# leospeidel/Colate

Measured on AMD Instinct MI355X. Metric: bootstrap replicates/sec to EM convergence, whole-genome SGDP mut, 20 epochs, higher is better.
Workload: dtype f64

## Files before the change

### colate_amd/csrc/em_kernel_impl.hpp

```cpp
#pragma once
#include <hip/hip_runtime.h>

#include <cstdlib>
#include <cstring>
#include <type_traits>

#include "em_kernels.h"
#include "em_math.hpp"

namespace {

constexpr int kWave = 64;
enum { O_W = 0, O_N, O_D, kNumBinArrays };
enum { G_LAM = 0, G_INV, G_XA, G_P, G_BETA, G_CS, G_S, G_PW, kNumGather };
constexpr int G_Q = kNumGather;
constexpr int num_gather_rows(int nch, bool tput) { return (nch >= 2 || !tput) ? kNumGather + 1 : kNumGather; }
constexpr int tail_scratch_arrays(int nch, bool tput) { return nch >= 2 ? (tput ? 3 : 6) : 0; }

__device__ __forceinline__ double readlane_d(double v, int lane) {
  int lo = __builtin_amdgcn_readlane(__double2loint(v), lane);
  int hi = __builtin_amdgcn_readlane(__double2hiint(v), lane);
  return __hiloint2double(hi, lo);
}

template <int CTRL, int ROW_MASK = 0xf, bool BOUND = false>
__device__ __forceinline__ double dpp_d(double old, double v) {
  int lo = __builtin_amdgcn_update_dpp(__double2loint(old), __double2loint(v), CTRL, ROW_MASK, 0xf, BOUND);
  int hi = __builtin_amdgcn_update_dpp(__double2hiint(old), __double2hiint(v), CTRL, ROW_MASK, 0xf, BOUND);
  return __hiloint2double(hi, lo);
}
constexpr int ROW_SHR1 = 0x111, ROW_SHR2 = 0x112, ROW_SHR4 = 0x114, ROW_SHR8 = 0x118;
constexpr int ROW_SHL1 = 0x101, ROW_SHL2 = 0x102, ROW_SHL4 = 0x104, ROW_SHL8 = 0x108;
constexpr int ROW_BCAST15 = 0x142, ROW_BCAST31 = 0x143, WAVE_SHR1 = 0x138, WAVE_SHL1 = 0x130;


__device__ __forceinline__ double wave_prefix_sum(double v, int rows = 4) {
  v += dpp_d<ROW_SHR1, 0xf, true>(0.0, v);
  v += dpp_d<ROW_SHR2, 0xf, true>(0.0, v);
  v += dpp_d<ROW_SHR4, 0xf, true>(0.0, v);
  v += dpp_d<ROW_SHR8, 0xf, true>(0.0, v);
  if (rows > 1) v += dpp_d<ROW_BCAST15, 0xa>(0.0, v);
  if (rows > 2) v += dpp_d<ROW_BCAST31, 0xc>(0.0, v);
  return v;
}
__device__ __forceinline__ double wave_suffix_sum(double v, int lane, int rows = 4) {
  v += dpp_d<ROW_SHL1, 0xf, true>(0.0, v);
  v += dpp_d<ROW_SHL2, 0xf, true>(0.0, v);
  v += dpp_d<ROW_SHL4, 0xf, true>(0.0, v);
  v += dpp_d<ROW_SHL8, 0xf, true>(0.0, v);
  if (rows > 1) {
    const double r1 = readlane_d(v, 16);
    double add = 0.0;
    if (rows > 2) {
      const double r2 = readlane_d(v, 32), r3 = readlane_d(v, 48);
      const double s23 = r2 + r3, s123 = r1 + s23;
      const int row = lane >> 4;
      add = row == 0 ? s123 : (row == 1 ? s23 : (row == 2 ? r3 : 0.0));
    } else {
      add = (lane >> 4) == 0 ? r1 : 0.0;
    }
    v = v + add;
  }
  return v;
}
__device__ __forceinline__ void wave_affine_scan(double& a, double& b, int rows = 4, const double* nosrc = nullptr) {
#define COLATE_AFF_STEP(CTRL, RM, BND, K)                                                                   \
  {                                                                                                         \
    const double as = nosrc ? dpp_d<CTRL, RM, true>(0.0, a) + nosrc[K] : dpp_d<CTRL, RM>(1.0, a);           \
    const double bs = dpp_d<CTRL, RM, BND>(0.0, b);                                                         \
    b = em::fma_(a, bs, b);                                                                                 \
    a = a * as;                                                                                             \
  }
  COLATE_AFF_STEP(ROW_SHR1, 0xf, true, 0)
  COLATE_AFF_STEP(ROW_SHR2, 0xf, true, 1)
  COLATE_AFF_STEP(ROW_SHR4, 0xf, true, 2)
  COLATE_AFF_STEP(ROW_SHR8, 0xf, true, 3)
#undef COLATE_AFF_STEP
  if (rows == 2) {
    const double bs = dpp_d<ROW_BCAST15, 0xa>(0.0, b);
    b = em::fma_(a, bs, b);
  }
#define COLATE_AFF_STEP2(CTRL, RM)                 \
  {                                                \
    const double as = dpp_d<CTRL, RM>(1.0, a);     \
    const double bs = dpp_d<CTRL, RM>(0.0, b);     \
    b = em::fma_(a, bs, b);                        \
    a = a * as;                                    \
  }
  if (rows > 2) COLATE_AFF_STEP2(ROW_BCAST15, 0xa)
  if (rows > 2) COLATE_AFF_STEP2(ROW_BCAST31, 0xc)
#undef COLATE_AFF_STEP2
}
constexpr int kAffSteps = 6;
__device__ __forceinline__ void wave_affine_scan_rates(double a, double (&am)[kAffSteps], int rows, const double* nosrc) {
  am[0] = a;
#define COLATE_AFF_STEP(CTRL, RM, K)                                                                        \
  {                                                                                                         \
    const double as = nosrc ? dpp_d<CTRL, RM, true>(0.0, a) + nosrc[K] : dpp_d<CTRL, RM>(1.0, a);           \
    a = a * as;                                                                                             \
    am[K + 1] = a;                                                                                          \
  }
  COLATE_AFF_STEP(ROW_SHR1, 0xf, 0)
  COLATE_AFF_STEP(ROW_SHR2, 0xf, 1)
  COLATE_AFF_STEP(ROW_SHR4, 0xf, 2)
// ... 16 lines not shown
  v = __builtin_fmax(v, dpp_d<ROW_SHL4, 0xf, true>(0.0, v));
  v = __builtin_fmax(v, dpp_d<ROW_SHL8, 0xf, true>(0.0, v));
  const double r1 = readlane_d(v, 16), r2 = readlane_d(v, 32), r3 = readlane_d(v, 48);
  const double m23 = __builtin_fmax(r2, r3), m123 = __builtin_fmax(r1, m23);
  const int row = lane >> 4;
  return __builtin_fmax(v, row == 0 ? m123 : (row == 1 ? m23 : (row == 2 ? r3 : 0.0)));
}
__device__ __forceinline__ double half_ulp_pos(double z) {
  const int ex = (__double2hiint(z) >> 20) & 0x7ff;
  return ex > 53 ? __hiloint2double((ex - 53) << 20, 0) : 0.0;
}

__device__ __forceinline__ double tail_hneg(double z, double& q) {
  const float a = __builtin_fminf(__builtin_fabsf((float)z), 30.0f);
  const float t = __builtin_amdgcn_rcpf(__builtin_fmaf(0.2316419f, a, 1.0f));
  float poly = __builtin_fmaf(t, 1.330274429f, -1.821255978f);
  poly = __builtin_fmaf(t, poly, 1.781477937f);
  poly = __builtin_fmaf(t, poly, -0.356563782f);
  poly = __builtin_fmaf(t, poly, 0.319381530f);
  poly = poly * t;
  const float phi = 0.3989422804f * __builtin_amdgcn_exp2f(-0.72134752f * (a * a));
  const float qa = phi * poly;
  const float base = __builtin_fmaxf(__builtin_fmaf(-a, qa, phi), 0.0f);
  q = z < 0.0 ? (double)(1.0f - qa) : (double)qa;
  return (z < 0.0 ? -z : 0.0) + (double)base;
}

#ifdef COLATE_EM_STAMPS
__device__ __forceinline__ unsigned long long stamp() {
  unsigned long long t;
  __builtin_amdgcn_sched_barrier(0);
  asm volatile("s_memtime %0\n\ts_waitcnt lgkmcnt(0)" : "=s"(t)::"memory");
  __builtin_amdgcn_sched_barrier(0);
  return t;
}
#define COLATE_STAMP(i)                     \
  {                                         \
    const unsigned long long now_ = stamp(); \
    st_acc[i] += now_ - st_prev;            \
    st_prev = now_;                         \
  }
#define COLATE_PSTAMP(i) pro_t[i] = stamp();
#else
#define COLATE_STAMP(i)
#define COLATE_PSTAMP(i)
#endif

#ifdef COLATE_ABL
#define COLATE_ABL_HAS(b) (((COLATE_ABL) >> (b)) & 1)
#else
#define COLATE_ABL_HAS(b) 0
#endif

#define COLATE_COLD() asm volatile("; cold path")
#define COLATE_STR2(x) #x
#define COLATE_STR(x) COLATE_STR2(x)

__device__ __forceinline__ bool finite_pos(double x) { return x > 0.0 && x < __builtin_inf(); }

__device__ __forceinline__ unsigned long long ballot64(bool p) { return __builtin_amdgcn_ballot_w64(p); }

__device__ __forceinline__ void wave_lds_fence() {
  __builtin_amdgcn_fence(__ATOMIC_RELEASE, "wavefront");
  __builtin_amdgcn_wave_barrier();
  __builtin_amdgcn_fence(__ATOMIC_ACQUIRE, "wavefront");
}

struct BinStat {
  double a_b, cnt, tk, tkn, dtk, da, db;
  double f1, f2, f4, f8;
  int kb, pos;
  bool live, last_bin, is_tail;
};
enum { BF_F1 = 1, BF_F2 = 2, BF_F4 = 4, BF_F8 = 8, BF_TAIL = 16, BF_INRANGE = 32, BF_KB_SHIFT = 8 };

constexpr int em_loop_pad(int mode, int nch, int erows, bool tput, int wpe) {
#ifdef COLATE_LOOP_PAD
  return (COLATE_LOOP_PAD) & 7;
#else
  (void)erows, (void)wpe;
  if (mode != 0) return 0;
#ifdef COLATE_EM_ILP_BUILD
  (void)tput;
  return nch == 1 ? (wpe == 2 ? 2 : 6) : 2;
#else
  (void)nch;
  if (!tput) return 6;
  return 4;
#endif
#endif
}

constexpr int em_loop_pad2(int mode, int nch, bool tput) {
#if defined(COLATE_EM_ILP_BUILD) && !defined(COLATE_LOOP_PAD)
  (void)mode, (void)nch, (void)tput;
  return -1;
#else
  (void)mode, (void)nch, (void)tput;
  return -1;
#endif
}

constexpr bool em_affine_split(int nch, bool tput, int wpe) {
#ifdef COLATE_AFFINE_SPLIT
  (void)nch, (void)tput, (void)wpe;
  return (COLATE_AFFINE_SPLIT) != 0;
#else
  return !tput && nch == 1 && wpe == 2;
#endif
}

template <int MODE, int NCH, int EROWS, bool TPUT, int WPE = 0>
__global__ __launch_bounds__(TPUT ? 2 * kWave : 2 * COLATE_EM_MAX_A, WPE ? WPE : ((NCH == 1) ? 3 : (NCH == 2 ? 2 : 1))) void em_kernel(ColateEmArgs p) {
  extern __shared__ double lds[];
  const int E = p.E, A = p.A;
  constexpr int EPAD = NCH * kWave;
  const int NBMAX = (A + kWave - 1) / kWave;
  const int AP = NBMAX * kWave;
  const int APZ = AP + 2;
  const int tid = threadIdx.x, lane = tid & 63;
  constexpr int kSlotShift = (NCH == 1) ? 0 : (NCH == 2 ? 1 : (NCH == 4 ? 2 : (NCH == 8 ? 3 : 4)));
  static_assert(NCH == 1 || NCH == 2 || NCH == 4 || NCH == 8 || NCH == 16, "NCH");
  auto ep_of = [&](int c) { return lane * NCH + c; };
  const int wave = __builtin_amdgcn_readfirstlane(tid >> 6);
  const int role = wave & 1;
  const int grp = wave >> 1;
  const int rep = blockIdx.x;

  double* s_t = lds;
  double* s_ep = s_t + EPAD + 1;
  constexpr int kRows = num_gather_rows(NCH, TPUT);
  double* s_out = s_ep + kRows * EPAD;
  double* s_nd = s_out + 2 * kNumBinArrays * APZ;
  double* s_cfail = s_nd + 4 * EPAD;
  double* s_cnt = s_cfail + 2 * APZ;
  double* s_ll = s_cnt + 2 * APZ;
  double* s_exptab = s_ll + 12;
  double* s_age = s_exptab + em::kExpTableDoubles;
  double* s_tscr = s_age + AP;
  int* s_kb = reinterpret_cast<int*>(s_tscr + tail_scratch_arrays(NCH, TPUT) * APZ);
  int* s_fail = s_kb + AP + 1;
  int* s_misc = s_fail + 8;
  int* s_bflags = s_misc + 4;

#ifdef COLATE_EM_TRACE
  unsigned long long trace_t0;
  asm volatile("s_memtime %0\n\ts_waitcnt lgkmcnt(0)" : "=s"(trace_t0)::"memory");
#endif
#ifdef COLATE_EM_STAMPS
  unsigned long long pro_t[10] = {0, 0, 0, 0, 0, 0, 0, 0, 0, 0};
#endif
  COLATE_PSTAMP(0)
  const double* epochs = p.epochs + (size_t)rep * p.epochs_stride;
  for (int i = tid; i < EPAD + 1; i += blockDim.x) s_t[i] = (i < E) ? epochs[i] : 0.0;
  for (int i = tid; i < kRows * EPAD + 2 * kNumBinArrays * APZ + 4 * EPAD + 4 * APZ; i += blockDim.x) s_ep[i] = 0.0;
  if (tid == 0) {
    s_misc[0] = A;
    s_misc[1] = 0;
    s_misc[2] = 0;
    s_misc[3] = 0;
  }
  if (tid < 8) {
    s_ll[tid] = 0.0;
    s_fail[tid] = 0;
  }
  if (tid < em::kExpTableDoubles) s_exptab[tid] = em::kExpTableDevice[tid];
  __syncthreads();
  COLATE_PSTAMP(1)
  for (int t = tid; t < AP; t += blockDim.x) {
    int kb = E;
    bool has_sh = false, has_ns = false;
    if (t < A) {
      const double a = p.age_grid[t];
      const double c1 = p.cnt_sh[(size_t)rep * A + t];
      const double c2 = p.cnt_ns[(size_t)rep * A + t];
      const double csh = (c1 > 0) ? c1 : 0.0;
      const double cns = (c2 > 0) ? c2 : 0.0;
      int first_gt = 0;
      for (int len = E; len > 0;) {
        const int half = len >> 1;
        if (!(a < s_t[first_gt + half])) {
          first_gt += half + 1;
          len -= half + 1;
        } else {
          len = half;
        }
      }
      kb = first_gt - 1;
      if (kb < 0) kb = 0;
      s_cnt[t] = csh;
      s_cnt[APZ + t] = cns;
      s_age[t] = a;
      has_sh = csh > 0;
      has_ns = cns > 0;
// ... 125 lines not shown
        const int half = len >> 1;
        if (s_kb[lo + half] < e) {
          lo += half + 1;
          len -= half + 1;
        } else {
          len = half;
        }
      }
      for (int len = A; len > 0;) {
        const int half = len >> 1;
        if (s_kb[hi + half] <= e) {
          hi += half + 1;
          len -= half + 1;
        } else {
          len = half;
        }
      }
      const int lo_c = lo < nzlo ? nzlo : (lo > nzhi ? nzhi : lo);
      n_before = lo_c - nzlo;
    }
    {
      int b0 = __builtin_amdgcn_readfirstlane(hi);
      if (b0 < nzlo) b0 = nzlo;
      for (int b = b0; b < nzhi; b += 8) {
        double v[8];
#pragma unroll
        for (int j = 0; j < 8; j++) v[j] = s_cnt[role * APZ + b + j];
#pragma unroll
        for (int j = 0; j < 8; j++) {
          c_later += (ep_on[c] && b + j >= hi && b + j < nzhi) ? v[j] : 0.0;
        }
      }
    }
    C0[c] = c_later;
    nlt[c] = n_before;
    const int clo = (lo > nzlo ? lo : nzlo) - nzlo, chi = (hi < nzhi ? hi : nzhi) - nzlo;
    seg_hi[c] = chi;
    slot0[c] = slot1[c] = slot2[c] = AP;
    row_x[c] = 1;
    row_hi[c] = 0;
    if (clo < chi) {
      const int r0 = clo >> 4, r1 = (chi - 1) >> 4;
      slot0[c] = (r0 * 16 + 15 < chi - 1) ? r0 * 16 + 15 : chi - 1;
      if (r1 > r0) slot1[c] = ((r0 + 1) * 16 + 15 < chi - 1) ? (r0 + 1) * 16 + 15 : chi - 1;
      if (r1 > r0 + 1) slot2[c] = ((r0 + 2) * 16 + 15 < chi - 1) ? (r0 + 2) * 16 + 15 : chi - 1;
      row_x[c] = r0 + 3;
      row_hi[c] = r1;
    }
  }
  if (role == 0) {
    const double from_below = dpp_d<WAVE_SHR1, 0xf, true>(0.0, C0[NCH - 1]);
#pragma unroll
    for (int c = 0; c < NCH; c++) {
      const double c_ge = (c == 0) ? (lane == 0 ? c_all : from_below) : C0[c - 1];
      eta_e[c] = dt_e[c] * (kIntegResidue * c_ge);
    }
  }
  bool more_rows[NCH];
  bool third_row = false;
#pragma unroll
  for (int c = 0; c < NCH; c++) {
    more_rows[c] = (ballot64(row_x[c] <= row_hi[c]) != 0);
    third_row |= (ballot64(slot2[c] != AP) != 0);
  }
  __syncthreads();
  COLATE_PSTAMP(6)
  if (!TPUT && grp >= NB) return;
  const bool leader = (grp == 0);
  constexpr bool kFreeBuild = !TPUT && NCH == 1 && WPE == 2;
  const int verdict_wave = (!TPUT && NB >= 2 && NCH != 2) ? (kFreeBuild ? 1 : 2) : 0;
  const bool tracker = (wave == verdict_wave);
  constexpr int erows = EROWS;
  constexpr bool kFree = kFreeBuild;
  double aff_nosrc[4] = {0.0, 0.0, 0.0, 0.0};
  if (kFree) {
    aff_nosrc[0] = (lane & 15) < 1 ? 1.0 : 0.0;
    aff_nosrc[1] = (lane & 15) < 2 ? 1.0 : 0.0;
    aff_nosrc[2] = (lane & 15) < 4 ? 1.0 : 0.0;
    aff_nosrc[3] = (lane & 15) < 8 ? 1.0 : 0.0;
  }
  const int p1b_wave = (kFree && NB >= 2) ? 3 : 1;
  const int nwave_live = 2 * NB;
  (void)nwave_live;

  int my_flags = 0;
  constexpr double kTinyNum = 1e-280;
  unsigned tr_min[NCH], tr_max[NCH];
  int tr_noisy = 0;
#pragma unroll
  for (int c = 0; c < NCH; c++) tr_min[c] = 0xffffffffu, tr_max[c] = 0u;
  constexpr double kNoisyRatio = 1.0e6;
  double noisy_thr[NCH];
#pragma unroll
  for (int c = 0; c < NCH; c++)
    noisy_thr[c] = (double)(ep_of(c)) <= s_ll[10] ? kNoisyRatio * (dt_e[c] * (kIntegResidue * (s_ll[8] + s_ll[9]))) : 0.0;
  unsigned long long prev_fail = 0;
  unsigned long long ep_mask[NCH];
#pragma unroll
  for (int c = 0; c < NCH; c++) ep_mask[c] = ballot64(ep_on[c]);
  const double thr = 1.0 - p.rel_tol;
  double ll = -__builtin_inf(), prev_ll = -__builtin_inf();
  int iter = 0;
  const int max_iter = (MODE == 1) ? 1 : p.max_iter;
  double* out_mine = s_out + role * kNumBinArrays * APZ;

#ifdef COLATE_EM_STAMPS
  unsigned long long st_acc[16] = {0, 0, 0, 0, 0, 0, 0, 0, 0, 0, 0, 0, 0, 0, 0, 0};
  COLATE_PSTAMP(7)
  unsigned long long st_prev = stamp();
#endif
  constexpr int kPad = em_loop_pad(MODE, NCH, EROWS, TPUT, WPE);
#define COLATE_PAD_CASE(n) \
  if constexpr (kPad == n) asm volatile(".p2align 6\n\t.rept " #n "\n\ts_nop 0\n\t.endr");
#define COLATE_LOOP_ANCHOR()                                            \
  {                                                                     \
    COLATE_PAD_CASE(0) COLATE_PAD_CASE(1) COLATE_PAD_CASE(2) COLATE_PAD_CASE(3) \
    COLATE_PAD_CASE(4) COLATE_PAD_CASE(5) COLATE_PAD_CASE(6) COLATE_PAD_CASE(7) \
  }
  bool last_pos = true;
  int lim = 0;
  constexpr bool kAssumeAbsorbing = kFree || TPUT;
  unsigned long long last_bit[NCH];
#pragma unroll
  for (int c = 0; c < NCH; c++) last_bit[c] = (((E - 1) & (NCH - 1)) == c) ? 1ull << (((E - 1) >> kSlotShift) & 63) : 0ull;
  auto last_rate_positive = [&]() {
    unsigned long long pos = 0;
#pragma unroll
    for (int c = 0; c < NCH; c++) pos |= ballot64(lam_e[c] > 0.0) & last_bit[c];
    return pos != 0ull;
  };
  const unsigned long long last_bit1 = 1ull << ((E - 1) & 63);
  if (kFree) last_pos = (ballot64(lam_e[0] > 0.0) & last_bit1) != 0ull;
  if (TPUT) last_pos = last_rate_positive();
  auto tail_due = [&](int it) {
#ifdef COLATE_TAIL_LATE256
    if (NCH >= 2) return it < 128 ? (it & (it - 1)) == 0 : (it < 512 ? (it & 127) == 0 : (it & 255) == 0);
#else
    if (NCH >= 2) return it < 128 ? (it & (it - 1)) == 0 : (it & 127) == 0;
#endif
    return (it & (it - 1)) == 0 || (!tail_trivial_prev && (it & 31) == 0);
  };
  auto tail_next_due = [&](int it) {
    if (it <= 1) return it;
    const int p2 = 1 << (32 - __builtin_clz((unsigned)(it - 1)));
#ifdef COLATE_TAIL_LATE256
    if (NCH >= 2) return it <= 128 ? p2 : (it <= 512 ? ((it + 127) & ~127) : ((it + 255) & ~255));
#else
    if (NCH >= 2) return it <= 128 ? p2 : ((it + 127) & ~127);
#endif
    const int m32 = (it + 31) & ~31;
    return (!tail_trivial_prev && m32 < p2) ? m32 : p2;
  };
  auto iteration = [&](auto role_c, auto leader_c, auto ll_c, auto track_c, auto refresh_c, auto p1_c) __attribute__((always_inline)) -> bool {
    COLATE_STAMP(7)
    constexpr int kRole = decltype(role_c)::value, kLeader = decltype(leader_c)::value, kNeedLL = decltype(ll_c)::value;
    constexpr int kTrack = decltype(track_c)::value;
    constexpr int kRefresh = decltype(refresh_c)::value;
    constexpr bool kSteady = (kNeedLL >= 0);
    const int ROLE = kRole < 0 ? role : kRole;
    const bool LEADER = kLeader < 0 ? leader : (kLeader != 0);
    constexpr bool kSplit = (kLeader >= 2);
    constexpr int kOwn = (kLeader == 3) ? 1 : 0;
    static_assert(!kSplit || NCH == 2, "the split is for two epochs per lane");
    auto own = [&](int c) { return !kSplit || c == kOwn; };
    constexpr int kP1 = decltype(p1_c)::value;
    const bool P1A = kP1 < 0 ? (ROLE == 0 && (kFree || LEADER)) : ((kP1 & 1) != 0);
    const bool P1B = kP1 < 0 ? (kFree ? wave == p1b_wave : (LEADER && ROLE == 1)) : ((kP1 & 2) != 0);
    constexpr bool CROSS = kFree;
    const bool need_ll = kNeedLL < 0 ? ((MODE == 1) || (iter >= p.min_iter) || (iter == max_iter - 1) || p.ll_trace != nullptr) : (kNeedLL != 0);
    double q_e[NCH], p_e[NCH], beta_e[NCH], S_e[NCH], omS_e[NCH], cs_e[NCH];
#pragma unroll
    for (int c = 0; c < NCH; c++) q_e[c] = p_e[c] = beta_e[c] = S_e[c] = omS_e[c] = cs_e[c] = 0.0;
    if ((P1A || P1B) && !COLATE_ABL_HAS(15)) {
      double x_e[NCH];
#pragma unroll
      for (int c = 0; c < NCH; c++) x_e[c] = lam_e[c] * dt_e[c];
      if (P1A) {
        double loc[NCH];
        loc[0] = 0.0;
#pragma unroll
        for (int c = 1; c < NCH; c++) loc[c] = loc[c - 1] + x_e[c - 1];
        const double tot = (NCH == 1) ? x_e[0] : loc[NCH - 1] + x_e[NCH - 1];
#if COLATE_ABL_HAS(11)
        const double incl = tot * 7.0;
#else
        const double incl = wave_prefix_sum(tot, erows);
#endif
        const double excl = dpp_d<WAVE_SHR1, 0xf, true>(0.0, incl);
#pragma unroll
        for (int c = 0; c < NCH; c++) cs_e[c] = (c == 0) ? excl : excl + loc[c];
      }
      COLATE_STAMP(8)
      if (P1A) {
#pragma unroll
        for (int c = 0; c < NCH; c++) {
          if (!own(c)) continue;
          const int e = ep_of(c);
#if COLATE_ABL_HAS(3)
          S_e[c] = 1.0 - cs_e[c] * 1e-3;
          omS_e[c] = cs_e[c] * 1e-3;
#else
          S_e[c] = em::em_exp_om_t<true>(cs_e[c], &omS_e[c], s_exptab);
#endif
          if (!kFree || LEADER) {
            s_ep[G_CS * EPAD + e] = cs_e[c];
            s_ep[G_S * EPAD + e] = S_e[c];
            s_ep[G_PW * EPAD + e] = omS_e[c];
          }
        }
      }
      if (P1B) {
#pragma unroll
        for (int c = 0; c < NCH; c++) {
          if (!own(c)) continue;
          const int e = ep_of(c);
#if COLATE_ABL_HAS(7)
          const double inv = 2.0e4 - lam_e[c];
#else
          const double inv = em::em_rcp_ieee(lam_e[c]);
#endif
          const bool valid = vstat[c] && (lam_e[c] > 0);
#if COLATE_ABL_HAS(4)
          const double qx = 1.0 - x_e[c];
#else
          const double qx = em::em_exp_t(-x_e[c], s_exptab);
#endif
          q_e[c] = (e < E - 1) ? qx : 0.0;
          p_e[c] = valid ? 1.0 - q_e[c] : 0.0;
          beta_e[c] = valid ? (t_e[c] + inv) - (tn_e[c] + inv) * q_e[c] : 0.0;
          s_ep[G_LAM * EPAD + e] = lam_e[c];
          if (!CROSS) {
            s_ep[G_INV * EPAD + e] = inv;
#if COLATE_ABL_HAS(7)
            s_ep[G_XA * EPAD + e] = (t_e[c] + inv) * lam_e[c];
#else
            s_ep[G_XA * EPAD + e] = em::em_div_known_rcp(t_e[c] + inv, inv, lam_e[c]);
#endif
          }
          s_ep[G_P * EPAD + e] = p_e[c];
          s_ep[G_BETA * EPAD + e] = beta_e[c];
          if (NCH >= 2 || kFree) s_ep[G_Q * EPAD + e] = q_e[c];
        }
      }
    }
    constexpr bool kHoist = em_affine_split(NCH, TPUT, WPE) && kSteady && kNeedLL == 0 && kRole == 1 && kLeader == 1;
    double aff_m[kAffSteps];
    if constexpr (kHoist) {
      double a = 1.0;
#pragma unroll
      for (int c = 0; c < NCH; c++) {
        if (!P1B) {
          const double qx = em::em_exp_t(-(lam_e[c] * dt_e[c]), s_exptab);
          q_e[c] = (ep_of(c) < E - 1) ? qx : 0.0;
        }
        const double qa = ep_on[c] ? q_e[c] : 1.0;
        a = (c == 0) ? qa : a * qa;
      }
      wave_affine_scan_rates(a, aff_m, erows, kFree ? aff_nosrc : nullptr);
#pragma unroll
      for (int k = 0; k < (erows > 2 ? 6 : (erows > 1 ? 5 : 4)); k++) asm volatile("" : "+v"(aff_m[k]));
    }
    double lk_pre = 0.0;
    if (!TPUT) {
      const int kq = bs0.kb < E ? bs0.kb : 0;
#pragma unroll
      for (int c = 0; c < NCH; c++) {
        const int lo = __builtin_amdgcn_ds_bpermute(((kq >> kSlotShift) & 63) << 2, __double2loint(lam_e[c]));
        const int hi = __builtin_amdgcn_ds_bpermute(((kq >> kSlotShift) & 63) << 2, __double2hiint(lam_e[c]));
        if (NCH == 1 || (kq & (NCH - 1)) == c) lk_pre = __hiloint2double(hi, lo);
      }
      asm volatile("" : "+v"(lk_pre));
    }
    double Sk_pre = 0.0, PWk_pre = 0.0, qd_pre = 0.0;
    if (kFree && ROLE == 0) {
      const int kq = bs0.kb < E ? bs0.kb : 0;
      const int s_lo = __builtin_amdgcn_ds_bpermute((kq & 63) << 2, __double2loint(S_e[0]));
      const int s_hi = __builtin_amdgcn_ds_bpermute((kq & 63) << 2, __double2hiint(S_e[0]));
      const int o_lo = __builtin_amdgcn_ds_bpermute((kq & 63) << 2, __double2loint(omS_e[0]));
      const int o_hi = __builtin_amdgcn_ds_bpermute((kq & 63) << 2, __double2hiint(omS_e[0]));
      Sk_pre = __hiloint2double(s_hi, s_lo);
      PWk_pre = __hiloint2double(o_hi, o_lo);
      qd_pre = em::em_exp_t(-(lk_pre * bs0.da), s_exptab);
    }
    COLATE_STAMP(9)
    bool absorbing = kAssumeAbsorbing && kSteady;
    if (!(kAssumeAbsorbing && kSteady)) {
      const int cl = (E - 1) & (NCH - 1), ll_ = (E - 1) >> kSlotShift;
#pragma unroll
      for (int c = 0; c < NCH; c++) {
        const unsigned long long pos = ballot64(lam_e[c] > 0.0);
        if (NCH == 1 || c == cl) absorbing = (pos >> ll_) & 1ull;
      }
    }
    if (!kFree || need_ll || !absorbing) __syncthreads();
    COLATE_STAMP(0)
    auto bin_terms = [&](const BinStat& bs, const double lk_own, const bool have_lk, const bool cross, const double Sk_in, const double PWk_in, const double qd_in) {
      const double a_b = bs.a_b, cnt = bs.cnt, tk = bs.tk, tkn = bs.tkn, dtk = bs.dtk, da = bs.da, db = bs.db;
      const double f1 = bs.f1, f2 = bs.f2, f4 = bs.f4, f8 = bs.f8;
      const int kb = bs.kb, pos = bs.pos;
      const bool live = bs.live, last_bin = bs.last_bin, is_tail = bs.is_tail;
      const int wslot = 2 * (pos >> 6) + ROLE;
      double o_w = 0, o_N = 0, o_D = 0, llp = 0.0;
      bool fail = false;
      unsigned long long fail_direct = 0;
      bool have_fail_direct = false;
      if (ROLE == 0 && !COLATE_ABL_HAS(12)) {
        const double lk = have_lk ? lk_own : s_ep[G_LAM * EPAD + kb];
        const bool lpos = lk > 0;
        const double ik = cross ? (lpos ? em::em_rcp_ieee(lk) : 0.0) : s_ep[G_INV * EPAD + kb];
        const double Sk = cross ? Sk_in : s_ep[G_S * EPAD + kb], PWk = cross ? PWk_in : s_ep[G_PW * EPAD + kb];
        const double Xak = cross ? em::em_div_known_rcp(tk + ik, ik, lk) : s_ep[G_XA * EPAD + kb];
#if COLATE_ABL_HAS(5)
        const double qd = 1.0 - lk * da;
#else
        const double qd = cross ? qd_in : em::em_exp_t(-(lk * da), s_exptab);
#endif
#if COLATE_ABL_HAS(8)
        const double Y = (a_b + ik) * lk;
#else
        const double Y = em::em_div_known_rcp(a_b + ik, ik, lk);
#endif
        const double Wp = (cross || lpos) ? Sk * (1.0 - qd) : 0.0;
        const double X = Xak - Y * qd;
        const double Vp = (cross || lpos) ? X * ik * Sk : 0.0;
        const double Sig = PWk + Wp;
        const bool fin = finite_pos(Sig), ok = live && fin;
        const double r = ok ? em::em_rcp(Sig) : 0.0;
        const double nk = Wp * r;
        double dk = Vp * r + (-tk * nk);
        dk = __builtin_fmax(dk, 0.0);
        o_w = cnt * r;
        o_N = cnt * nk;
        o_D = cnt * dk;
        fail_direct = ballot64(live) & ~ballot64(fin);
        have_fail_direct = true;
        if (need_ll) {
          COLATE_COLD();
          llp = ok ? cnt * em::em_log(Sig) : 0.0;
        }
      } else if (ROLE == 1 && !COLATE_ABL_HAS(12)) {
        const double lk = have_lk ? lk_own : s_ep[G_LAM * EPAD + kb];
        const double ik = cross ? em::em_rcp_ieee(lk) : s_ep[G_INV * EPAD + kb];
        const bool lpos = lk > 0;
        auto neg_cs_age = [&]() {
          const double ck = s_ep[G_CS * EPAD + kb];
          const double ck1 = ck + lk * da;
          return -(ck1 + lk * (a_b - a_b));
        };
#if COLATE_ABL_HAS(6)
        const double u = 1.0 - lk * db;
#else
        const double u = em::em_exp_t(-(lk * db), s_exptab);
#endif
        const double pn = 1.0 - u;
        const double bn = lpos ? (a_b + ik) - (tkn + ik) * u : 0.0;
        {
          double dk = bn + (-tk * pn + dtk * (1.0 - pn));
          dk = __builtin_fmax(dk, 0.0);
          o_w = cnt * u;
          o_N = cnt * pn;
          o_D = cnt * dk;
          if (need_ll) {
            COLATE_COLD();
            llp = live ? cnt * neg_cs_age() : 0.0;
          }
        }
        if (__builtin_expect(!absorbing, 0)) {
          COLATE_COLD();
          o_w = o_N = o_D = llp = 0.0;
          if (live) {
            const double Gk1 = 1.0 - em::em_exp_t(-s_ep[G_CS * EPAD + E - 1] + s_ep[G_CS * EPAD + kb + 1], s_exptab);
            const double SigN = pn + u * Gk1;
            if (finite_pos(SigN)) {
              const double rr = 1.0 / SigN;
              const double nk = pn * rr;
              double dk = bn * rr + (-tk * nk + dtk * (1.0 - nk));
              dk = __builtin_fmax(dk, 0.0);
              o_w = cnt * (u * rr);
              o_N = cnt * nk;
              o_D = cnt * dk;
              llp = cnt * (neg_cs_age() + em::em_log(SigN));
            } else {
              fail = true;
            }
          }
        }
        if (__builtin_expect(ballot64(last_bin && live) != 0, 0)) {
          COLATE_COLD();
          if (last_bin && live) {
// ... 358 lines not shown
      if (MODE == 1 && ep_on[c]) {
        if (N_e[c] != N_e[c] || D_e[c] != D_e[c]) my_flags |= COLATE_FLAG_NAN;
        if (N_e[c] < 0.0 || D_e[c] < 0.0) my_flags |= COLATE_FLAG_NEG;
      }
    }
    COLATE_STAMP(13)
    if (need_ll) {
      COLATE_COLD();
      ll = ((s_ll[0] + s_ll[1]) + (s_ll[2] + s_ll[3])) + ((s_ll[4] + s_ll[5]) + (s_ll[6] + s_ll[7]));
      if (kNeedLL < 0 && p.ll_trace && tid == 0 && iter < p.ll_trace_cap) p.ll_trace[(size_t)rep * p.ll_trace_cap + iter] = ll;
    }
    if (MODE == 1) {
      if (wave == 0) {
#pragma unroll
        for (int c = 0; c < NCH; c++) {
          if (ep_on[c]) {
            p.out_num[(size_t)rep * E + ep_of(c)] = N_e[c];
            p.out_den[(size_t)rep * E + ep_of(c)] = D_e[c];
          }
        }
      }
      return true;
    }
    if (!COLATE_ABL_HAS(14)) {
      double cand[NCH];
      bool self[NCH];
      unsigned long long keep[NCH];
      unsigned long long cpm[NCH];
#pragma unroll
      for (int c = 0; c < NCH; c++) {
        const bool copy = (N_e[c] == 0);
        {
#if COLATE_ABL_HAS(10)
          double qn = N_e[c] * 1e-4 + D_e[c] * 1e-9;
#else
          double qn = N_e[c] / D_e[c];
#endif
          qn = em::max_c(qn, p.rate_floor);
          cand[c] = (!copy && D_e[c] != 0) ? qn : lam_e[c];
        }
        const unsigned long long zero_n = __builtin_amdgcn_fcmp(N_e[c], 0.0, 1 );
        keep[c] = ep_mask[c] & ~zero_n;
        cpm[c] = ep_mask[c] & zero_n;
        self[c] = ep_on[c] && !copy;
      }
      unsigned long long bad = (NCH == 1) ? 0ull : (cpm[0] & ~((cpm[NCH - 1] << 1) | 1ull));
#pragma unroll
      for (int c = 0; c < NCH; c++) {
        bad |= cpm[c] & (cpm[c] + 1ull);
        if (c > 0) bad |= cpm[c] & ~cpm[c - 1];
      }
      if (kTrack < 0 ? tracker : (kTrack != 0)) {
#pragma unroll
        for (int c = 0; c < NCH; c++) {
          const unsigned nh = (unsigned)__double2hiint(N_e[c]);
          tr_min[c] = nh < tr_min[c] ? nh : tr_min[c];
          tr_max[c] = nh > tr_max[c] ? nh : tr_max[c];
          tr_noisy |= (ep_on[c] && N_e[c] != 0.0 && D_e[c] < noisy_thr[c] && cand[c] > p.rate_floor) ? 1 : 0;
        }
      }
      if (__builtin_expect(bad == 0, 1)) {
#pragma unroll
        for (int c = 0; c < NCH; c++) lam_e[c] = self[c] ? cand[c] : 0.0;
      } else {
        COLATE_COLD();
        unsigned long long any_keep = 0;
        double lastc = 0.0;
#pragma unroll
        for (int c = 0; c < NCH; c++) {
          any_keep |= keep[c];
          lastc = self[c] ? cand[c] : lastc;
        }
        const unsigned long long below = any_keep & ((1ull << lane) - 1ull);
        const int src = below ? 63 - __builtin_clzll(below) : 0;
        const double from_lanes = __shfl(lastc, src, 64);
        double prev = below ? from_lanes : 0.0;
#pragma unroll
        for (int c = 0; c < NCH; c++) {
          lam_e[c] = ep_on[c] ? (self[c] ? cand[c] : prev) : 0.0;
          prev = self[c] ? cand[c] : prev;
        }
      }
    }
    if (kAssumeAbsorbing && kSteady) {
      lim = (kFree ? ((ballot64(lam_e[0] > 0.0) & last_bit1) != 0ull) : last_rate_positive()) ? lim : 0;
      asm volatile("" : "+s"(lim));
    }
    COLATE_STAMP(5)
    bool stop = false;
    if (kNeedLL != 0 && iter > p.min_iter) {
      COLATE_COLD();
      stop = (ll / prev_ll > thr);
    }
    prev_ll = ll;
    return stop;
  };
  bool stopped = false;
  if constexpr (NCH <= 4) if (MODE == 0 && p.ll_trace == nullptr) {
    int n_steady = p.min_iter < max_iter - 1 ? p.min_iter : max_iter - 1;
    if (n_steady < 0) n_steady = 0;
    using C0 = std::integral_constant<int, 0>;
    using C1 = std::integral_constant<int, 1>;
    using CR = std::integral_constant<int, -1>;
#define COLATE_STEADY(R, L, T, P)                             \
  {                                                           \
    lim = n_steady;                                           \
    COLATE_LOOP_ANCHOR()                                      \
    do {                                                      \
      iteration(R{}, L{}, C0{}, T{}, C0{}, P{});              \
    } while (__builtin_expect(++iter < lim, 1));              \
    if (kAssumeAbsorbing && lim == 0) last_pos = false;                  \
  }
#define COLATE_STEADY_B(R, L, T, P)                                                    \
  while (iter < n_steady && last_pos) {                                                \
    if (tail_due(iter)) {                                                              \
      lim = n_steady;                                                                  \
      iteration(R{}, L{}, C0{}, T{}, C1{}, P{});                                       \
      ++iter;                                                                          \
      if (kAssumeAbsorbing && lim == 0) last_pos = false;                                         \
      if (iter >= n_steady || !last_pos) break;                                        \
    }                                                                                  \
    lim = tail_next_due(iter);                                                         \
    if (lim > n_steady) lim = n_steady;                                                \
    COLATE_LOOP_ANCHOR()                                                               \
    while (__builtin_expect(iter < lim, 1)) {                                          \
      iteration(R{}, L{}, C0{}, T{}, C0{}, P{});                                       \
      ++iter;                                                                          \
    }                                                                                  \
    if (kAssumeAbsorbing && lim == 0) last_pos = false;                                           \
  }
    bool any_more_rows = false;
#pragma unroll
    for (int c = 0; c < NCH; c++) any_more_rows |= more_rows[c];
#define COLATE_STEADY_LL(R, L, T, P)                          \
  if (last_pos) {                                             \
    lim = max_iter;                                           \
    COLATE_LOOP_ANCHOR()                                      \
    for (; iter < lim; iter++) {                              \
      if (iteration(R{}, L{}, C1{}, T{}, C0{}, P{})) {        \
        stopped = true;                                       \
        break;                                                \
      }                                                       \
    }                                                         \
    if (kAssumeAbsorbing && lim == 0) last_pos = false;                  \
  }
#define COLATE_STEADY_LL_B(R, L, T, P)                                                 \
  while (iter < max_iter && !stopped && last_pos) {                                    \
    if (tail_due(iter)) {                                                              \
      lim = max_iter;                                                                  \
      if (iteration(R{}, L{}, C1{}, T{}, C1{}, P{})) {                                 \
        stopped = true;                                                                \
        break;                                                                         \
      }                                                                                \
      ++iter;                                                                          \
      if (kAssumeAbsorbing && lim == 0) last_pos = false;                                         \
      if (iter >= max_iter || !last_pos) break;                                        \
    }                                                                                  \
    lim = tail_next_due(iter);                                                         \
    if (lim > max_iter) lim = max_iter;                                                \
    COLATE_LOOP_ANCHOR()                                                               \
    for (; iter < lim; iter++) {                                                       \
      if (iteration(R{}, L{}, C1{}, T{}, C0{}, P{})) {                                 \
        stopped = true;                                                                \
        break;                                                                         \
      }                                                                                \
    }                                                                                  \
    if (kAssumeAbsorbing && lim == 0) last_pos = false;                                           \
  }
#ifndef COLATE_LL_MAX_NCH
#define COLATE_LL_MAX_NCH 2
#endif
#ifdef COLATE_NO_LL_LOOPS
#define COLATE_BOTH(R, L, T, P)                               \
  {                                                           \
    if (iter < n_steady && last_pos) COLATE_STEADY(R, L, T, P); \
  }
#define COLATE_BOTH_B(R, L, T, P)                             \
  {                                                           \
    COLATE_STEADY_B(R, L, T, P)                               \
  }
#else
#define COLATE_BOTH(R, L, T, P)                               \
  {                                                           \
    if (iter < n_steady && last_pos) COLATE_STEADY(R, L, T, P); \
    if constexpr (NCH <= COLATE_LL_MAX_NCH) COLATE_STEADY_LL(R, L, T, P) \
  }
#define COLATE_BOTH_B(R, L, T, P)                             \
  {                                                           \
    COLATE_STEADY_B(R, L, T, P)                               \
// ... 211 lines not shown
```

### colate_amd/csrc/em_math.hpp

```cpp
#pragma once

#if defined(__HIPCC__) || defined(__HIP__)
#define EM_HD __host__ __device__ __forceinline__
#else
#define EM_HD inline
#endif

namespace em {

EM_HD double fma_(double a, double b, double c) { return __builtin_fma(a, b, c); }

EM_HD double fma_cc(double c1, double x, double c0) {
#if defined(__HIP_DEVICE_COMPILE__)
  double d;
  asm("v_fma_f64 %0, %1, %2, %3" : "=v"(d) : "s"(c1), "v"(x), "v"(c0));
  return d;
#else
  return __builtin_fma(c1, x, c0);
#endif
}
EM_HD double max_c(double x, double lo) {
#if defined(__HIP_DEVICE_COMPILE__)
  double d;
  asm("v_max_f64 %0, %1, %2" : "=v"(d) : "v"(x), "s"(lo));
// ... 56 lines not shown
  return o;
}

EM_HD double em_exp(double x) {
  const double xc = max_c(x, -1100.0);
  const ExpParts o = em_exp_parts(xc);
  return __builtin_ldexp(o.y, o.ki);
}

EM_HD double em_exp_om(double x, double* one_minus) {
  const double xc = max_c(x, -1100.0);
  const ExpParts o = em_exp_parts(xc);
  const double y = __builtin_ldexp(o.y, o.ki);
  *one_minus = (o.ki == 0) ? -(o.rh + o.tp) : 1.0 - y;
  return y;
}

#define EM_EXP_TABLE_VALUES \
  0x1.0000000000000p+0, 0x0.0p+0, \
  0x1.059b0d3158574p+0, 0x1.d73e2a475b465p-55, \
  0x1.0b5586cf9890fp+0, 0x1.8a62e4adc610bp-54, \
  0x1.11301d0125b51p+0, -0x1.6c51039449b3ap-54, \
  0x1.172b83c7d517bp+0, -0x1.19041b9d78a76p-55, \
  0x1.1d4873168b9aap+0, 0x1.e016e00a2643cp-54, \
  0x1.2387a6e756238p+0, 0x1.9b07eb6c70573p-54, \
  0x1.29e9df51fdee1p+0, 0x1.612e8afad1255p-55, \
  0x1.306fe0a31b715p+0, 0x1.6f46ad23182e4p-55, \
  0x1.371a7373aa9cbp+0, -0x1.63aeabf42eae2p-54, \
  0x1.3dea64c123422p+0, 0x1.ada0911f09ebcp-55, \
  0x1.44e086061892dp+0, 0x1.89b7a04ef80d0p-59, \
  0x1.4bfdad5362a27p+0, 0x1.d4397afec42e2p-56, \
  0x1.5342b569d4f82p+0, -0x1.07abe1db13cadp-55, \
  0x1.5ab07dd485429p+0, 0x1.6324c054647adp-54, \
  0x1.6247eb03a5585p+0, -0x1.383c17e40b497p-54, \
  0x1.6a09e667f3bcdp+0, -0x1.bdd3413b26456p-54, \
  0x1.71f75e8ec5f74p+0, -0x1.16e4786887a99p-55, \
  0x1.7a11473eb0187p+0, -0x1.41577ee04992fp-55, \
  0x1.82589994cce13p+0, -0x1.d4c1dd41532d8p-54, \
  0x1.8ace5422aa0dbp+0, 0x1.6e9f156864b27p-54, \
  0x1.93737b0cdc5e5p+0, -0x1.75fc781b57ebcp-57, \
  0x1.9c49182a3f090p+0, 0x1.c7c46b071f2bep-56, \
  0x1.a5503b23e255dp+0, -0x1.d2f6edb8d41e1p-54, \
  0x1.ae89f995ad3adp+0, 0x1.7a1cd345dcc81p-54, \
  0x1.b7f76f2fb5e47p+0, -0x1.5584f7e54ac3bp-56, \
  0x1.c199bdd85529cp+0, 0x1.11065895048ddp-55, \
  0x1.cb720dcef9069p+0, 0x1.503cbd1e949dbp-56, \
  0x1.d5818dcfba487p+0, 0x1.2ed02d75b3707p-55, \
  0x1.dfc97337b9b5fp+0, -0x1.1a5cd4f184b5cp-54, \
  0x1.ea4afa2a490dap+0, -0x1.e9c23179c2893p-54, \
  0x1.f50765b6e4540p+0, 0x1.9d3e12dd8a18bp-54
constexpr int kExpTableDoubles = 64;
#if defined(__HIPCC__) || defined(__HIP__)
static __device__ const double kExpTableDevice[kExpTableDoubles] = {EM_EXP_TABLE_VALUES};
#endif
static const double kExpTableHost[kExpTableDoubles] = {EM_EXP_TABLE_VALUES};

struct ExpTab {
  double th, tl, p;
  int e;
};
EM_HD ExpTab em_exp_tab_parts(double xc, const double* tab) {
  const double INVLN2N = 0x1.71547652b82fep+5;
  const double LN2N_HI = 0x1.62e42fefa0000p-6;
  const double LN2N_MID = 0x1.cf79abc9e0000p-45;
  const double SHIFT = 0x1.8p52;
  ExpTab o;
  const double kd = fma_(xc, INVLN2N, SHIFT);
  const int ki = em_lo32(kd);
  const double k = kd - SHIFT;
  const double r = fma_(-k, LN2N_MID, fma_(-k, LN2N_HI, xc));
  const int j = ki & 31;
  o.e = ki >> 5;
  o.th = tab[2 * j];
  o.tl = tab[2 * j + 1];
  const double r2 = r * r;
  const double a = fma_cc(0x1.5555555555555p-3, r, 0x1.0000000000000p-1);
  const double b = fma_cc(0x1.1111111111111p-7, r, 0x1.5555555555555p-5);
  const double c = fma_cc(0x1.a01a01a01a01ap-13, r, 0x1.6c16c16c16c17p-10);
  const double r4 = r2 * r2;
  const double q = fma_(c, r4, fma_(b, r2, a));
  o.p = fma_(r2, q, r);
  return o;
}
EM_HD double em_exp_t(double x, const double* tab) {
#ifdef COLATE_EXP_SERIES
  (void)tab;
  return em_exp(x);
#endif
  const double xc = max_c(x, -1100.0);
  const ExpTab o = em_exp_tab_parts(xc, tab);
  return __builtin_ldexp(o.th + fma_(o.th, o.p, o.tl), o.e);
}
template <bool NEG = false>
EM_HD double em_exp_om_t(double x, double* one_minus, const double* tab) {
#ifdef COLATE_EXP_SERIES
  (void)tab;
  return em_exp_om(NEG ? -x : x, one_minus);
#endif
  const double xc = NEG ? max_c_neg(x, -1100.0) : max_c(x, -1100.0);
  const ExpTab o = em_exp_tab_parts(xc, tab);
  const double yh = __builtin_ldexp(o.th, o.e);
  const double yl = __builtin_ldexp(fma_(o.th, o.p, o.tl), o.e);
  *one_minus = (1.0 - yh) - yl;
  return yh + yl;
}

EM_HD double em_rcp(double x) {
#if defined(__HIP_DEVICE_COMPILE__)
  double y = __builtin_amdgcn_rcp(x);
  double e = fma_(-x, y, 1.0);
  y = fma_(y, e, y);
  e = fma_(-x, y, 1.0);
  y = fma_(y, e, y);
  return y;
#else
  return 1.0 / x;
#endif
}

EM_HD double em_rcp_ieee(double x) {
#if defined(__HIP_DEVICE_COMPILE__)
  double y = __builtin_amdgcn_rcp(x);
  double e = fma_(-x, y, 1.0);
  y = fma_(y, e, y);
  e = fma_(-x, y, 1.0);
  y = fma_(y, e, y);
  const double r = fma_(-x, y, 1.0);
  const double q = fma_(r, y, y);
  return __builtin_amdgcn_div_fixup(q, x, 1.0);
#else
  return 1.0 / x;
#endif
}

EM_HD double em_div_known_rcp(double n, double d, double y) {
  double q = n * y;
  double r = fma_(-q, d, n);
  q = fma_(r, y, q);
  r = fma_(-q, d, n);
  q = fma_(r, y, q);
  return q;
}

EM_HD double em_log(double x) {
  const double LN2_HI = 0x1.62e42fefa39efp-1;
  const double LN2_LO = 0x1.abc9e3b39803fp-56;
  if (!(x > 0.0)) return (x == 0.0) ? -__builtin_inf() : __builtin_nan("");
  if (x > 0x1.fffffffffffffp+1023) return x;
  int m;
  double f = __builtin_frexp(x, &m);
  if (f < 0x1.6a09e667f3bcdp-1) {
    f = f + f;
    m = m - 1;
  }
  double z = f - 1.0;
  double s = z / (2.0 + z);
  double w = s * s;
  double q = 0x1.642c8590b2164p-4;
  q = fma_(q, w, 0x1.8618618618618p-4);
  q = fma_(q, w, 0x1.af286bca1af28p-4);
  q = fma_(q, w, 0x1.e1e1e1e1e1e1ep-4);
  q = fma_(q, w, 0x1.1111111111111p-3);
  q = fma_(q, w, 0x1.3b13b13b13b14p-3);
  q = fma_(q, w, 0x1.745d1745d1746p-3);
  q = fma_(q, w, 0x1.c71c71c71c71cp-3);
  q = fma_(q, w, 0x1.2492492492492p-2);
  q = fma_(q, w, 0x1.999999999999ap-2);
  q = fma_(q, w, 0x1.5555555555555p-1);
  double hfsq = s * z;
  double logf = z - (hfsq - (s * w) * q);
  double dm = (double)m;
  return fma_(dm, LN2_HI, logf + dm * LN2_LO);
}

}
```

Measured before the change: 112,300.

## Hand-schedule role-A front of EM iteration, interleaving prefix scan with exp/rcp

Measured after the change: 121,400 (median of 6 runs). 1.08x the previous value.

```diff
diff --git a/colate_amd/csrc/em_kernel_impl.hpp b/colate_amd/csrc/em_kernel_impl.hpp
--- a/colate_amd/csrc/em_kernel_impl.hpp
+++ b/colate_amd/csrc/em_kernel_impl.hpp
@@ -20,6 +20,12 @@
 __device__ __forceinline__ double readlane_d(double v, int lane) {
   int lo = __builtin_amdgcn_readlane(__double2loint(v), lane);
   int hi = __builtin_amdgcn_readlane(__double2hiint(v), lane);
+  return __hiloint2double(hi, lo);
+}
+
+__device__ __forceinline__ double bpermute_d(int addr, double v) {
+  const int lo = __builtin_amdgcn_ds_bpermute(addr, __double2loint(v));
+  const int hi = __builtin_amdgcn_ds_bpermute(addr, __double2hiint(v));
   return __hiloint2double(hi, lo);
 }
 
@@ -202,7 +208,7 @@
   if (mode != 0) return 0;
 #ifdef COLATE_EM_ILP_BUILD
   (void)tput;
-  return nch == 1 ? (wpe == 2 ? 2 : 6) : 2;
+  return nch == 1 ? (wpe == 2 ? (erows == 2 ? 6 : 2) : 6) : 2;
 #else
   (void)nch;
   if (!tput) return 6;
@@ -230,6 +236,16 @@
 #endif
 }
 
+constexpr bool em_role_a_front(int nch, bool tput, int wpe) {
+#if defined(COLATE_EXP_SERIES) || defined(COLATE_ABL)
+  (void)nch, (void)tput, (void)wpe;
+  return false;
+#elif defined(COLATE_ROLE_A_FRONT)
+  return (COLATE_ROLE_A_FRONT) != 0 && !tput && nch == 1 && wpe == 2;
+#else
+  return !tput && nch == 1 && wpe == 2;
+#endif
+}
 template <int MODE, int NCH, int EROWS, bool TPUT, int WPE = 0>
 __global__ __launch_bounds__(TPUT ? 2 * kWave : 2 * COLATE_EM_MAX_A, WPE ? WPE : ((NCH == 1) ? 3 : (NCH == 2 ? 2 : 1))) void em_kernel(ColateEmArgs p) {
   extern __shared__ double lds[];
@@ -521,6 +537,14 @@
   const int p1b_wave = (kFree && NB >= 2) ? 3 : 1;
   const int nwave_live = 2 * NB;
   (void)nwave_live;
+  constexpr bool kFrontBuild = kFree && em_role_a_front(NCH, TPUT, WPE);
+  double lk_carry = 0.0, x_carry = 0.0;
+  const int bp_k = kFrontBuild ? ((bs0.kb < E ? bs0.kb : 0) & 63) << 2 : 0;
+  unsigned long long live_mask = 0;
+  if constexpr (kFrontBuild) {
+    live_mask = ballot64(bs0.live);
+    asm volatile("" : "+s"(live_mask));
+  }
 
   int my_flags = 0;
   constexpr double kTinyNum = 1e-280;
@@ -610,7 +634,82 @@
     double q_e[NCH], p_e[NCH], beta_e[NCH], S_e[NCH], omS_e[NCH], cs_e[NCH];
 #pragma unroll
     for (int c = 0; c < NCH; c++) q_e[c] = p_e[c] = beta_e[c] = S_e[c] = omS_e[c] = cs_e[c] = 0.0;
-    if ((P1A || P1B) && !COLATE_ABL_HAS(15)) {
+    constexpr bool kFront = kFrontBuild && kSteady && kNeedLL == 0 && kRole == 0;
+    double head_ik = 0.0, head_Xak = 0.0, head_Y = 0.0, head_Sk = 0.0, head_PWk = 0.0, head_qd = 0.0;
+    if constexpr (kFront) {
+      static_assert(NCH == 1, "one epoch per lane");
+#define COLATE_CUT() __builtin_amdgcn_sched_barrier(0);
+#define COLATE_PIN(x) asm volatile("" : "+v"(x));
+      const double lk = lk_carry;
+      double v = x_carry;
+      v += dpp_d<ROW_SHR1, 0xf, true>(0.0, v);
+      COLATE_CUT()
+      const double xc2 = em::max_c(-(lk * bs0.da), -1100.0);
+      double zero15 = 0.0;
+      double y2 = em::em_rcp_ieee_seed(lk);
+      COLATE_PIN(zero15) COLATE_PIN(y2) COLATE_CUT()
+      v += dpp_d<ROW_SHR2, 0xf, true>(0.0, v);
+      COLATE_CUT()
+      em::ExpK k2 = em::em_exp_tab_k(xc2);
+      unsigned long long lpos_mask = __builtin_amdgcn_fcmp(lk, 0.0, 2 );
+      COLATE_PIN(k2.kd) COLATE_PIN(k2.k) asm volatile("" : "+s"(lpos_mask)); COLATE_CUT()
+      v += dpp_d<ROW_SHR4, 0xf, true>(0.0, v);
+      COLATE_CUT()
+      const int ki2 = em::em_lo32(k2.kd);
+      int e2 = ki2 >> 5, j2 = 2 * (ki2 & 31);
+      double r2 = em::em_exp_tab_r(xc2, k2.k);
+      COLATE_PIN(e2) COLATE_PIN(j2) COLATE_PIN(r2) COLATE_CUT()
+      v += dpp_d<ROW_SHR8, 0xf, true>(0.0, v);
+      COLATE_CUT()
+      const double th2 = s_exptab[j2], tl2 = s_exptab[j2 + 1];
+      COLATE_CUT()
+      if (erows > 1) {
+        v += dpp_d<ROW_BCAST15, 0xa>(zero15, v);
+        COLATE_CUT()
+      }
+      double ik_all = em::em_rcp_ieee_refine(lk, y2);
+      COLATE_PIN(ik_all) COLATE_CUT()
+      if (erows > 2) {
+        head_ik = __builtin_amdgcn_inverse_ballot_w64(lpos_mask) ? ik_all : 0.0;
+        COLATE_PIN(head_ik) COLATE_CUT()
+        v += dpp_d<ROW_BCAST31, 0xc>(0.0, v);
+        COLATE_CUT()
+      }
+      cs_e[0] = dpp_d<WAVE_SHR1, 0xf, true>(0.0, v);
+      COLATE_STAMP(8)
+      const double xc1 = em::max_c_neg(cs_e[0], -1100.0);
+      COLATE_CUT()
+      if (erows <= 2) {
+        head_ik = __builtin_amdgcn_inverse_ballot_w64(lpos_mask) ? ik_all : 0.0;
+        COLATE_PIN(head_ik) COLATE_CUT()
+      }
+      em::ExpK k1 = em::em_exp_tab_k(xc1);
+      const int ki1 = em::em_lo32(k1.kd);
+      const int e1 = ki1 >> 5, j1 = 2 * (ki1 & 31);
+      double r1 = em::em_exp_tab_r(xc1, k1.k);
+      const double th1 = s_exptab[j1], tl1 = s_exptab[j1 + 1];
+      COLATE_CUT()
+      double p1 = em::em_exp_tab_poly(r1);
+      double p2 = em::em_exp_tab_poly(r2);
+      COLATE_PIN(p1) COLATE_PIN(p2) COLATE_CUT()
+      S_e[0] = em::em_exp_tab_value_om(th1, tl1, p1, e1, &omS_e[0]);
+      if (LEADER) {
+        const int e = ep_of(0);
+        s_ep[G_CS * EPAD + e] = cs_e[0];
+        s_ep[G_S * EPAD + e] = S_e[0];
+        s_ep[G_PW * EPAD + e] = omS_e[0];
+      }
+      head_Sk = bpermute_d(bp_k, S_e[0]);
+      head_PWk = bpermute_d(bp_k, omS_e[0]);
+      COLATE_CUT()
+      head_Xak = em::em_div_known_rcp(bs0.tk + head_ik, head_ik, lk);
+      head_Y = em::em_div_known_rcp(bs0.a_b + head_ik, head_ik, lk);
+      head_qd = em::em_exp_tab_value(th2, tl2, p2, e2);
+      COLATE_PIN(head_Xak) COLATE_PIN(head_Y) COLATE_CUT()
+#undef COLATE_PIN
+#undef COLATE_CUT
+    }
+    if constexpr (!kFront) if ((P1A || P1B) && !COLATE_ABL_HAS(15)) {
       double x_e[NCH];
 #pragma unroll
       for (int c = 0; c < NCH; c++) x_e[c] = lam_e[c] * dt_e[c];
@@ -700,7 +799,7 @@
       for (int k = 0; k < (erows > 2 ? 6 : (erows > 1 ? 5 : 4)); k++) asm volatile("" : "+v"(aff_m[k]));
     }
     double lk_pre = 0.0;
-    if (!TPUT) {
+    if constexpr (!kFront) if (!TPUT) {
       const int kq = bs0.kb < E ? bs0.kb : 0;
 #pragma unroll
       for (int c = 0; c < NCH; c++) {
@@ -711,7 +810,11 @@
       asm volatile("" : "+v"(lk_pre));
     }
     double Sk_pre = 0.0, PWk_pre = 0.0, qd_pre = 0.0;
-    if (kFree && ROLE == 0) {
+    if constexpr (kFront) {
+      lk_pre = lk_carry;
+      Sk_pre = head_Sk, PWk_pre = head_PWk, qd_pre = head_qd;
+    }
+    if constexpr (!kFront) if (kFree && ROLE == 0) {
       const int kq = bs0.kb < E ? bs0.kb : 0;
       const int s_lo = __builtin_amdgcn_ds_bpermute((kq & 63) << 2, __double2loint(S_e[0]));
       const int s_hi = __builtin_amdgcn_ds_bpermute((kq & 63) << 2, __double2hiint(S_e[0]));
@@ -743,7 +846,26 @@
       bool fail = false;
       unsigned long long fail_direct = 0;
       bool have_fail_direct = false;
-      if (ROLE == 0 && !COLATE_ABL_HAS(12)) {
+      if constexpr (kFront) {
+        const double ik = head_ik, Sk = Sk_in, PWk = PWk_in, Xak = head_Xak, qd = qd_in, Y = head_Y;
+        const double Wp = Sk * (1.0 - qd);
+        const double X = Xak - Y * qd;
+        const double Vp = X * ik * Sk;
+        const double Sig = PWk + Wp;
+        unsigned long long fin_mask;
+        asm("v_cmp_class_f64 %0, %1, %2" : "=s"(fin_mask) : "v"(Sig), "v"(0x180));
+        const bool ok = __builtin_amdgcn_inverse_ballot_w64(live_mask & fin_mask);
+        const double r = ok ? em::em_rcp(Sig) : 0.0;
+        const double nk = Wp * r;
+        double dk = Vp * r + (-tk * nk);
+        dk = __builtin_fmax(dk, 0.0);
+        o_w = cnt * r;
+        o_N = cnt * nk;
+        o_D = cnt * dk;
+        fail_direct = live_mask & ~fin_mask;
+        have_fail_direct = true;
+        (void)a_b, (void)live, (void)lk_own;
+      } else if (ROLE == 0 && !COLATE_ABL_HAS(12)) {
         const double lk = have_lk ? lk_own : s_ep[G_LAM * EPAD + kb];
         const bool lpos = lk > 0;
         const double ik = cross ? (lpos ? em::em_rcp_ieee(lk) : 0.0) : s_ep[G_INV * EPAD + kb];
@@ -1268,6 +1390,11 @@
         }
       }
     }
+    if constexpr (kFront) {
+      x_carry = lam_e[0] * dt_e[0];
+      asm volatile("" : "+v"(x_carry));
+      lk_carry = bpermute_d(bp_k, lam_e[0]);
+    }
     if (kAssumeAbsorbing && kSteady) {
       lim = (kFree ? ((ballot64(lam_e[0] > 0.0) & last_bit1) != 0ull) : last_rate_positive()) ? lim : 0;
       asm volatile("" : "+s"(lim));
@@ -1291,6 +1418,7 @@
 #define COLATE_STEADY(R, L, T, P)                             \
   {                                                           \
     lim = n_steady;                                           \
+    if constexpr (kFrontBuild && R::value == 0) x_carry = lam_e[0] * dt_e[0], lk_carry = bpermute_d(bp_k, lam_e[0]); \
     COLATE_LOOP_ANCHOR()                                      \
     do {                                                      \
       iteration(R{}, L{}, C0{}, T{}, C0{}, P{});              \
diff --git a/colate_amd/csrc/em_math.hpp b/colate_amd/csrc/em_math.hpp
--- a/colate_amd/csrc/em_math.hpp
+++ b/colate_amd/csrc/em_math.hpp
@@ -162,6 +162,33 @@
   o.p = fma_(r2, q, r);
   return o;
 }
+struct ExpK {
+  double kd, k;
+};
+EM_HD ExpK em_exp_tab_k(double xc) {
+  ExpK o;
+  o.kd = fma_(xc, 0x1.71547652b82fep+5, 0x1.8p52);
+  o.k = o.kd - 0x1.8p52;
+  return o;
+}
+EM_HD double em_exp_tab_r(double xc, double k) { return fma_(-k, 0x1.cf79abc9e0000p-45, fma_(-k, 0x1.62e42fefa0000p-6, xc)); }
+EM_HD double em_exp_tab_poly(double r) {
+  const double r2 = r * r;
+  const double a = fma_cc(0x1.5555555555555p-3, r, 0x1.0000000000000p-1);
+  const double b = fma_cc(0x1.1111111111111p-7, r, 0x1.5555555555555p-5);
+  const double c = fma_cc(0x1.a01a01a01a01ap-13, r, 0x1.6c16c16c16c17p-10);
+  const double r4 = r2 * r2;
+  const double q = fma_(c, r4, fma_(b, r2, a));
+  return fma_(r2, q, r);
+}
+EM_HD double em_exp_tab_value(double th, double tl, double p, int e) { return __builtin_ldexp(th + fma_(th, p, tl), e); }
+EM_HD double em_exp_tab_value_om(double th, double tl, double p, int e, double* one_minus) {
+  const double yh = __builtin_ldexp(th, e);
+  const double yl = __builtin_ldexp(fma_(th, p, tl), e);
+  *one_minus = (1.0 - yh) - yl;
+  return yh + yl;
+}
+
 EM_HD double em_exp_t(double x, const double* tab) {
 #ifdef COLATE_EXP_SERIES
   (void)tab;
@@ -210,6 +237,28 @@
   return __builtin_amdgcn_div_fixup(q, x, 1.0);
 #else
   return 1.0 / x;
+#endif
+}
+
+EM_HD double em_rcp_ieee_seed(double x) {
+#if defined(__HIP_DEVICE_COMPILE__)
+  return __builtin_amdgcn_rcp(x);
+#else
+  return 1.0 / x;
+#endif
+}
+EM_HD double em_rcp_ieee_refine(double x, double y) {
+#if defined(__HIP_DEVICE_COMPILE__)
+  double e = fma_(-x, y, 1.0);
+  y = fma_(y, e, y);
+  e = fma_(-x, y, 1.0);
+  y = fma_(y, e, y);
+  const double r = fma_(-x, y, 1.0);
+  const double q = fma_(r, y, y);
+  return __builtin_amdgcn_div_fixup(q, x, 1.0);
+#else
+  (void)x;
+  return y;
 #endif
 }
 
```
